# GATB/leon

Hardware: AMD Instinct MI355X
Metric: compressed input MB/s (DNA encode path) (higher is better)
Workload: dtype u64

## Files before the change

### include/leon_dna.h

```cpp
#ifndef LEON_DNA_H
#define LEON_DNA_H

#include <stddef.h>
#include <stdint.h>

#ifdef __cplusplus
extern "C" {
#endif

#define LEON_DNA_ABI_VERSION 5

enum {
    LEON_OK = 0,
    LEON_E_INVALID = -1,
    LEON_E_NO_DEVICE = -2,
    LEON_E_HIP = -3,
    LEON_E_STATE = -4,
    LEON_E_OVERFLOW = -5,
    LEON_E_SINK = -6
};

typedef struct leon_dna_ctx leon_dna_ctx;

typedef struct leon_dna_cfg {
// ... 14 lines not shown
#define LEON_F_DICT_ON_DEVICE 2u

typedef int (*leon_block_sink)(void* user, uint64_t block_id, const uint8_t* payload, uint64_t size,
                               uint32_t n_reads);

typedef struct leon_dna_stats {
    uint64_t n_reads, n_bases, n_blocks, n_anchors, n_no_anchor, n_symbols, payload_bytes;
    uint64_t resolve_rounds, resolve_windows;
    float ms_pack, ms_resolve, ms_sort, ms_walk, ms_symbols, ms_rangecoder, ms_d2h, ms_total;
    uint32_t walk_launches, reserved;
    float ms_anchor_wait, ms_chain_busy;
    float ms_exchange, ms_exchange_call, ms_emulated, ms_emulated_lookups;
    uint64_t xch_words_sent, xch_words_received, walk_reads;
    uint64_t resolve_chain_reads, resolve_chain_windows;
    float ms_resolve_chain, ms_gather_call;
} leon_dna_stats;

int  leon_dna_ctx_create(const leon_dna_cfg* cfg, leon_dna_ctx** out);
void leon_dna_ctx_destroy(leon_dna_ctx* ctx);
const char* leon_last_error(const leon_dna_ctx* ctx);
int  leon_dna_abi_version(void);

int leon_dna_bloom_nbytes(const leon_dna_ctx* ctx, uint64_t* nbytes);
int leon_dna_bloom_upload(leon_dna_ctx* ctx, const uint8_t* bits, uint64_t nbytes);
int leon_dna_bloom_download(leon_dna_ctx* ctx, uint8_t* bits, uint64_t nbytes);
int leon_dna_bloom_clear(leon_dna_ctx* ctx);
int leon_dna_bloom_insert(leon_dna_ctx* ctx, const uint64_t* kmers, uint64_t n);
int leon_dna_bloom_insert_device(leon_dna_ctx* ctx, const uint64_t* d_kmers, uint64_t n);
int leon_dna_bloom_device_ptr(leon_dna_ctx* ctx, void** d_bits, uint64_t* nbytes);
int leon_dna_bloom_upload_device(leon_dna_ctx* ctx, const uint8_t* d_bits, uint64_t nbytes);
// ... 167 lines not shown
```

### leon_amd/capi.py

```python
import ctypes as C
import os
import threading

import numpy as np

_HERE = os.path.dirname(os.path.abspath(__file__))

ABI_VERSION = 5
HEADER_TEXT_DEVICE_CAP = 4096
LEON_F_KEEP_TRACE = 1
LEON_F_DICT_ON_DEVICE = 2


class LeonDnaError(RuntimeError):
    def __init__(self, code, msg):
        super().__init__("leon_dna error %d: %s" % (code, msg))
        self.code = code


def lib_path():
    return os.path.join(_HERE, "lib", "libleon_dna.so")


class _Cfg(C.Structure):
    _fields_ = [("struct_size", C.c_uint32), ("kmer_size", C.c_uint32), ("reads_per_block", C.c_uint32),
                ("bloom_n_hash", C.c_uint32), ("bloom_block_nbits", C.c_uint32), ("device_id", C.c_int32),
                ("bloom_tai", C.c_uint64), ("random_values", C.POINTER(C.c_uint64)), ("resolve_window", C.c_uint64),
                ("flags", C.c_uint32), ("reserved", C.c_uint32)]


class Stats(C.Structure):
    _fields_ = [(n, C.c_uint64) for n in ("n_reads", "n_bases", "n_blocks", "n_anchors", "n_no_anchor", "n_symbols",
                                           "payload_bytes", "resolve_rounds", "resolve_windows")] + \
               [(n, C.c_float) for n in ("ms_pack", "ms_resolve", "ms_sort", "ms_walk", "ms_symbols", "ms_rangecoder",
                                         "ms_d2h", "ms_total")] + \
               [("walk_launches", C.c_uint32), ("reserved", C.c_uint32), ("ms_anchor_wait", C.c_float),
                ("ms_chain_busy", C.c_float)] + \
               [(n, C.c_float) for n in ("ms_exchange", "ms_exchange_call", "ms_emulated", "ms_emulated_lookups")] + \
               [(n, C.c_uint64) for n in ("xch_words_sent", "xch_words_received", "walk_reads", "resolve_chain_reads", "resolve_chain_windows")] + \
               [("ms_resolve_chain", C.c_float), ("ms_gather_call", C.c_float)]

    def as_dict(self):
        return {n: getattr(self, n) for n, _ in self._fields_ if not n.startswith("reserved")}


SINK = C.CFUNCTYPE(C.c_int, C.c_void_p, C.c_uint64, C.POINTER(C.c_uint8), C.c_uint64, C.c_uint32)
EXCHANGE = C.CFUNCTYPE(C.c_int, C.c_void_p, C.c_void_p, C.POINTER(C.c_uint64), C.c_uint32, C.POINTER(C.c_void_p), C.POINTER(C.c_uint64))
XCH_OFF, XCH_BY_ANCHOR, XCH_EMULATE = 0, 1, 2
GATHER = C.CFUNCTYPE(C.c_int, C.c_void_p, C.c_void_p, C.c_uint64, C.c_uint32)

PIECE_SINK = C.CFUNCTYPE(C.c_int, C.c_void_p, C.c_uint64, C.c_void_p, C.c_uint64)


class RecordLayout(C.Structure):
    _fields_ = [("struct_size", C.c_uint32), ("lead", C.c_uint8), ("fastq", C.c_uint8), ("plus_kind", C.c_uint8), ("reserved", C.c_uint8),
# ... 1058 lines not shown
```

### leon_amd/csrc/capi.hip

```cpp
#include "../../include/leon_dna.h"
#include "kernels.h"
#include "host_rc.h"
#include "staging.h"
#include "host_blocks.h"
#include "host_bgzf.h"

#include "prim.h"

#include <algorithm>
#include <atomic>
#include <chrono>
#include <cstdio>
#include <cstdlib>
#include <cstring>
#include <functional>
#include <mutex>
#include <string>
#include <thread>
#include <vector>

using namespace leon;

namespace {

// ... 80 lines not shown
    DevBuf anchor_kmers;
    AnchorDictWorker* anchor_worker = nullptr;
    double anchor_wait_ms = 0;
    std::vector<uint8_t> dict_device_out;
    uint64_t next_read = 0, next_block = 0;
    uint32_t shard_rank = 0, shard_world = 1;
    uint32_t xch_mode = LEON_XCH_OFF;
    leon_exchange_fn xch_fn = nullptr; void* xch_user = nullptr;
    leon_gather_fn gather_fn = nullptr; void* gather_user = nullptr;
    DevBuf xch_slot, xch_off, xch_evoff, xch_events, xch_send, xch_split, xch_res;
    DevBuf resolve_trace;
    DevBuf round_hist;
    DevBuf wcache;
    DevBuf chain_cnt, chain_own, chain_ins, chain_rows, chain_ent, chain_trace, chain_dep, chain_xdep, chain_om, chain_late;
    std::vector<hipEvent_t> chain_ev;
    DevBuf hb_recs[2], hb_recoff, hb_state;
    uint64_t* h_recs = nullptr; size_t h_recs_cap = 0;
    hipStream_t copy_stream = nullptr;
    std::vector<hipEvent_t> hb_ev;
    std::vector<HostBlockCoder> hb_coders;
    uint64_t* h_anchor[2] = {nullptr, nullptr}; size_t h_anchor_cap = 0;
    bool partial_seen = false, finished = false;
    uint64_t hdr_next_read = 0, hdr_next_block = 0;
    bool hdr_partial_seen = false;
    DevBuf hdr_first;
    const uint64_t* walk_keys = nullptr;
    uint32_t fbits_log2 = FBITS_LOG2_DEFAULT;
    bool poisoned = false;
    DevBuf in_bases, in_off, slot_off, packed, nmask, rlen, ncount;
    DevBuf status, hit_pos, hit_slot, cand_pos, cand_slot, anchor_pos, anchor_addr, flags, sort_key, ins_flag, rank;
// ... 461 lines not shown
    }
    CREATE_CHK(c->fbits.ensure((1ull << c->fbits_log2) / 8));
    CREATE_CHK(hipMemsetAsync(c->fbits.p, 0, (1ull << c->fbits_log2) / 8, c->stream));
    CREATE_CHK(hipStreamSynchronize(c->stream));
#undef CREATE_CHK
    c->anchor_worker = new AnchorDictWorker(cfg->kmer_size);
    *out = c;
    return LEON_OK;
}

void leon_dna_ctx_destroy(leon_dna_ctx* c) {
    if (!c) return;
    delete c->anchor_worker;
    (void)hipSetDevice(c->device);
    if (c->stream) (void)hipStreamSynchronize(c->stream);
    dict_free(c->D);
    DevBuf* bufs[] = { &c->anchor_kmers, &c->in_bases, &c->in_off, &c->slot_off, &c->packed, &c->nmask, &c->rlen, &c->ncount,
                       &c->status, &c->hit_pos, &c->hit_slot, &c->cand_pos, &c->cand_slot, &c->anchor_pos, &c->anchor_addr,
                       &c->flags, &c->sort_key, &c->ins_flag, &c->rank, &c->ulist0, &c->ulist1, &c->counters, &c->cub_tmp,
                       &c->sort_key2, &c->perm, &c->perm2, &c->events, &c->prev, &c->sym_off, &c->syms, &c->blk_begin,
                       &c->out_off, &c->out_size, &c->rc_out, &c->rc_scratch, &c->dst_off, &c->payload, &c->errflag, &c->nerr, &c->wbits, &c->fbits, &c->pbits, &c->hdr_first, &c->dc_cache, &c->dc_out, &c->dc_pay, &c->dc_len, &c->dc_pool, &c->dc_scr,
                       &c->xch_slot, &c->xch_off, &c->xch_evoff, &c->xch_events, &c->xch_send, &c->xch_split, &c->xch_res, &c->round_hist, &c->resolve_trace, &c->hb_recs[0], &c->hb_recs[1], &c->hb_recoff, &c->hb_state };
    for (DevBuf* b : bufs) b->release();
    if (c->d_bloom) (void)hipFree(c->d_bloom);
    if (c->d_rv16) (void)hipFree(c->d_rv16);
    if (c->d_nkeys) (void)hipFree(c->d_nkeys);
    if (c->h_payload) (void)hipHostFree(c->h_payload);
    if (c->h_rb) (void)hipHostFree(c->h_rb);
    for (auto& b : c->h_anchor) if (b) (void)hipHostFree(b);
    if (c->h_recs) (void)hipHostFree(c->h_recs);
    for (auto& e : c->hb_ev) (void)hipEventDestroy(e);
    if (c->copy_stream) (void)hipStreamDestroy(c->copy_stream);
    for (auto& e : c->ev) if (e) (void)hipEventDestroy(e);
    for (auto& e : c->pack_ev) (void)hipEventDestroy(e);
    for (auto& e : c->chain_ev) (void)hipEventDestroy(e);
    if (c->stream) (void)hipStreamDestroy(c->stream);
    delete c;
}

int leon_dna_bloom_nbytes(const leon_dna_ctx* c, uint64_t* n) {
    if (!c || !n) return LEON_E_INVALID;
    *n = c->bloom_nchar;
    return LEON_OK;
}
int leon_dna_bloom_upload(leon_dna_ctx* c, const uint8_t* bits, uint64_t n) {
    if (!c || !bits) return LEON_E_INVALID;
    if (n != c->bloom_nchar) return fail(c, LEON_E_INVALID, "bloom_upload: size differs from leon_dna_bloom_nbytes");
    HIPCHK(c, hipSetDevice(c->device));
    HIPCHK(c, staged_h2d(c->device, c->d_bloom, bits, n));
    return LEON_OK;
// ... 72 lines not shown
}
int leon_dna_bloom_contains(leon_dna_ctx* c, const uint64_t* kmers, uint64_t n, uint8_t* out) {
    return bloom_query(c, kmers, n, 0, out);
}

static uint64_t first_window(uint64_t window) { return std::min<uint64_t>(window, 1ull << 17); }
static uint64_t group_end(uint64_t a, uint64_t n, uint64_t window) {
    if (a == 0) return std::min(n, first_window(window));
    return std::min(n, a + 8 * std::min<uint64_t>(window, 1ull << 20));
}

namespace {

struct EncodeKnobs {
    uint32_t rounds_ahead, rounds_max;
    uint32_t chain_chunk;
    bool xch_lookups, walk_cache;
    long walk_cache_log2, walk_hop_log2;
    bool trace_step, trace_resolve, trace_chain;
};
long env_num(const char* name, long dflt) { const char* e = getenv(name); return e ? atol(e) : dflt; }
EncodeKnobs read_encode_knobs() {
    const char* rounds = getenv("LEON_RESOLVE_ROUNDS");
    const long ahead = env_num("LEON_RESOLVE_ROUNDS", 0), most = rounds && strchr(rounds, ':') ? atol(strchr(rounds, ':') + 1) : 0;
    const long chunk = env_num("LEON_CHAIN_CHUNK", 0), hop = env_num("LEON_WALK_HOP_LOG2", 4);
    EncodeKnobs K{};
    K.rounds_ahead = ahead >= 1 && ahead <= 32 ? (uint32_t)ahead : 3u;
    K.rounds_max = std::max<uint32_t>(K.rounds_ahead, most >= 1 && most <= 62 ? (uint32_t)most : 9u);
    K.chain_chunk = chunk >= 1 && chunk <= (1l << CHAIN_LOG2) ? (uint32_t)chunk : 1u << CHAIN_LOG2;
    K.xch_lookups = env_num("LEON_XCH_LOOKUPS", 1) != 0; K.walk_cache = env_num("LEON_WALK_CACHE", 1) != 0;
    K.walk_cache_log2 = env_num("LEON_WALK_CACHE_LOG2", 0); K.walk_hop_log2 = hop >= 1 && hop <= 8 ? hop : 4;
    K.trace_step = getenv("LEON_TRACE_STEP"); K.trace_resolve = getenv("LEON_TRACE_RESOLVE"); K.trace_chain = getenv("LEON_TRACE_CHAIN");
    return K;
}

struct EncodeBatch {
    leon_dna_ctx* const c;
    const uint8_t* const d_bases; const uint64_t* const d_off; const uint64_t n, first_read_index; const leon_block_sink sink; void* const user;
    Upload* const up; const uint64_t* const up_off;
    const uint64_t* const walk_keys = c->walk_keys;
    const EncodeKnobs knobs = read_encode_knobs();
    const std::chrono::steady_clock::time_point t_enter = std::chrono::steady_clock::now();
    const hipStream_t s = c->stream;
    const uint32_t rpb = c->cfg.reads_per_block, k = c->cfg.kmer_size;
    uint64_t n_blocks = 0, off_first = 0, off_last = 0, n_slots = 0, W = 0, KW = 0;
    ReadsDev R{}; ResolveDev V{};
    uint64_t packed_upto = 0; uint32_t n_pack_ev = 0;
    static constexpr uint32_t kRoundsMore = 2, kHist = 64;
    uint32_t* counters = nullptr; uint32_t* lists[2] = {nullptr, nullptr}; uint32_t* d_hist = nullptr; unsigned long long* d_trace = nullptr;
    size_t scan_tmp = 0;
    struct Pending { int buf = -1; uint64_t n = 0; } pending;
    int anchor_buf = 0; bool share_lookups = false;
    uint32_t hint = 0;
    uint32_t n_chain_ev = 0;
    float lk_call_ms = 0, lk_emul_ms = 0;
    Share sh{}; uint64_t nl_bases = 0; bool by_anchor = false;
    WalkCache wc{nullptr, 0, 28, 0};
    std::vector<uint64_t> slice_at, rank_r0, send_counts, send_at; size_t scan_n = 0;
    void mark(const char* what) const {
        if (knobs.trace_step) fprintf(stderr, "[leon step] %-34s %8.2f ms\n", what, std::chrono::duration<double, std::milli>(std::chrono::steady_clock::now() - t_enter).count());
    }
    float ms(int a, int b) const { float v = 0; (void)hipEventElapsedTime(&v, c->ev[a], c->ev[b]); return v; }
    int start() {
        c->stats = leon_dna_stats{}; c->walk_keys = nullptr;
        HIPCHK(c, hipMemcpyAsync(c->h_rb + 0, d_off, 8, hipMemcpyDeviceToHost, s));
        HIPCHK(c, hipMemcpyAsync(c->h_rb + 1, d_off + n, 8, hipMemcpyDeviceToHost, s));
        HIPCHK(c, spin_sync(s));
        off_first = c->h_rb[0]; off_last = c->h_rb[1];
        if (off_last < off_first) return fail(c, LEON_E_INVALID, "offsets are not monotonic");
        n_blocks = (n + rpb - 1) / rpb;
        HIPCHK(c, hipEventRecord(c->ev[0], s));
        HIPCHK(c, c->slot_off.ensure((n + 1) * 8));
// ... 106 lines not shown
            }
            HIPCHK(c, hipStreamSynchronize(s));
            lk_emul_ms += ms_since(t_l0);
        }
        launch_lookup_apply(s, R, c->D, V, w0, w1, s0, s1, first_read_index, xres, lists[0], counters);
        return LEON_OK;
    }
    int fixpoint_rounds(uint64_t w0, uint64_t w1, uint32_t& cnt0) {
        int cur = 0;
        uint32_t n_hist = 1;
        bool first_wait = true;
        for (uint32_t ahead = knobs.rounds_ahead;; ahead = kRoundsMore) {
            for (uint32_t r = 0; r < ahead && n_hist < kHist; r++) {
                const int nxt = cur ^ 1;
                const uint32_t h = std::max<uint32_t>(hint >> (2 * (n_hist - 1) < 31 ? 2 * (n_hist - 1) : 31), 4096);
                HIPCHK(c, hipMemsetAsync(counters + nxt, 0, 4, s));
                launch_check(s, R, c->D, V, first_read_index, lists[cur], counters + cur, h, lists[nxt], counters + nxt);
                HIPCHK(c, hipMemcpyAsync(d_hist + n_hist, counters + nxt, 4, hipMemcpyDeviceToDevice, s));
                launch_reset_tent(s, c->D, V, lists[cur], counters + cur, h);
                launch_propose(s, c->D, V, first_read_index, lists[nxt], counters + nxt, h);
                cur = nxt; n_hist++;
            }
            HIPCHK(c, hipMemcpyAsync(c->h_rb + 8, d_hist, n_hist * 4, hipMemcpyDeviceToHost, s));
            HIPCHK(c, hipMemcpyAsync(c->h_rb + 1, c->D.err, 4, hipMemcpyDeviceToHost, s));
            HIPCHK(c, spin_sync(s));
            if (first_wait) { hand_over(); first_wait = false; }
            if (const int derr = (int)(uint32_t)c->h_rb[1]) {
                HIPCHK(c, hipMemsetAsync(c->D.err, 0, 4, s));
                return fail(c, LEON_E_STATE, derr == 2 ? "the look-ups gathered from the other ranks do not fit this rank's reads or dictionary (were all ranks fed the same batches?)"
                                                       : "anchor dictionary: a two-word key stayed half-written (a stalled wave); batch abandoned");
            }
            const uint32_t* hist = reinterpret_cast<const uint32_t*>(c->h_rb + 8);
            cnt0 = hist[0];
            for (uint32_t r = 1; r < n_hist; r++)
                if (hist[r - 1] > 0 && hist[r] >= hist[r - 1]) return fail(c, LEON_E_STATE, "anchor resolution made no progress (internal error)");
            const uint32_t cnt = hist[n_hist - 1];
            const bool halving = n_hist >= 2 && 2ull * hist[n_hist - 1] <= hist[n_hist - 2];
            if (cnt == 0 || !halving || n_hist - 1 >= knobs.rounds_max || n_hist + kRoundsMore > kHist) {
                for (uint32_t r = 1; r < n_hist; r++) if (hist[r - 1] > 0) c->stats.resolve_rounds++;
                return cnt ? chain_tail(cnt, w0, w1, lists[cur ^ 1]) : LEON_OK;
            }
        }
    }
    int chain_tail(uint32_t left, uint64_t w0, uint64_t w1, uint32_t* clist) {
        if (int rc = event_pair(c, c->chain_ev, n_chain_ev)) return rc;
        HIPCHK(c, hipEventRecord(c->chain_ev[2 * n_chain_ev], s));
        uint32_t* rank = c->rank.as<uint32_t>();
        launch_chain_flags(s, V, w0, w1, V.ins_flag);
        HIPCHK(c, prim::ExclusiveSum(c->cub_tmp.p, scan_tmp, V.ins_flag, rank, w1 - w0, s));
        launch_chain_compact(s, V, w0, w1, rank, clist);
// ... 10 lines not shown
            uint64_t* rows = c->chain_rows.as<uint64_t>();
            uint32_t* cnt = c->chain_cnt.as<uint32_t>(); uint32_t* own = c->chain_own.as<uint32_t>();
            unsigned long long* om = c->chain_om.as<unsigned long long>(); unsigned long long* late = c->chain_late.as<unsigned long long>();
            unsigned long long* dep = c->chain_dep.as<unsigned long long>(); unsigned long long* xdep = c->chain_xdep.as<unsigned long long>();
            size_t rows_tmp = 0;
            HIPCHK(c, prim::ExclusiveSum(nullptr, rows_tmp, rows, rows, nG + 1, s));
            if (rows_tmp > c->cub_tmp.cap) { HIPCHK(c, hipStreamSynchronize(s)); if (int rc = ensure_cub(c, std::max(rows_tmp, scan_tmp))) return rc; }
            launch_chain_prep(s, false, R, c->D, V, first_read_index, w0, clist + c0, nc, c0, rank, cnt, own, nullptr, nullptr, nullptr, nullptr, nullptr, nullptr);
            launch_chain_tables(s, cnt, own, nc, rows, om, late);
            HIPCHK(c, prim::ExclusiveSum(c->cub_tmp.p, rows_tmp, rows, rows, nG + 1, s));
            HIPCHK(c, hipMemcpyAsync(c->h_rb + 0, rows + nG, 8, hipMemcpyDeviceToHost, s));
            HIPCHK(c, spin_sync(s));
            const uint64_t total_rows = c->h_rb[0];
            HIPCHK(c, c->chain_ent.ensure(std::max<uint64_t>(total_rows, 1) * 64 * 4)); uint32_t* ent = c->chain_ent.as<uint32_t>();
            launch_chain_prep(s, true, R, c->D, V, first_read_index, w0, clist + c0, nc, c0, rank, cnt, own, rows, ent, om, late, dep, xdep);
            if (launch_chain_seq(s, nc, cnt, own, dep, xdep, rows, ent, c->chain_ins.as<unsigned long long>(), d_ctrace))
                return fail(c, LEON_E_HIP, "the sequential resolution pass could not be launched (its LDS request was refused)");
            launch_chain_apply(s, c->D, V, first_read_index, clist + c0, nc, c->chain_ins.as<unsigned long long>(), k);
            HIPCHK(c, hipGetLastError());
        }
        { const uint32_t c_last = (left - 1) / CH * CH; launch_chain_repropose(s, c->D, V, first_read_index, clist + c_last, left - c_last, nullptr, 0); }
        HIPCHK(c, hipEventRecord(c->chain_ev[2 * n_chain_ev + 1], s));
        n_chain_ev++;
        c->stats.resolve_chain_reads += left; c->stats.resolve_chain_windows++;
        if (knobs.trace_chain) {
            unsigned long long t[8];
            HIPCHK(c, hipStreamSynchronize(s));
            HIPCHK(c, hipMemcpy(t, d_ctrace, sizeof t, hipMemcpyDeviceToHost));
            float cms = 0; (void)hipEventElapsedTime(&cms, c->chain_ev[2 * n_chain_ev - 2], c->chain_ev[2 * n_chain_ev - 1]);
            fprintf(stderr, "[leon chain] window [%llu, %llu): %u reads left by the rounds; %llu steps of 64, %.2f ballot iterations and %.1f entry rows per step, %llu inserters; %.2f ms; per step the settler waited %.0f (tester: %.0f), settled + published %.0f ticks of s_memtime\n",
// ... 29 lines not shown
            if (w0 == 0) {
                HIPCHK(c, spin_sync(s));
                hand_over();
                mark("first window's anchors to the chain");
            }
        }
        c->n_anchors += n_new;
        return LEON_OK;
    }
    void hand_over() {
        if (pending.buf < 0) return;
        std::vector<uint64_t> fresh(c->h_anchor[pending.buf], c->h_anchor[pending.buf] + pending.n * KW);
        c->anchor_worker->push(std::move(fresh));
        pending.buf = -1;
    }
    int take_share() {
        sh = share_of(c, n);
        uint64_t off_r0 = off_first, off_r1 = off_last;
        if (c->shard_world > 1) {
            HIPCHK(c, hipMemcpy(&off_r0, d_off + sh.r0, 8, hipMemcpyDeviceToHost));
            HIPCHK(c, hipMemcpy(&off_r1, d_off + sh.r0 + sh.nl, 8, hipMemcpyDeviceToHost));
        }
        nl_bases = off_r1 - off_r0;
        R.ev_origin = sh.r0;
        c->stats.n_reads = sh.nl; c->stats.n_bases = nl_bases; c->stats.n_blocks = sh.nbl; c->stats.n_anchors = c->n_anchors;
        c->last_n = n; c->last_bases = nl_bases; c->last_d_bases = d_bases; c->last_d_off = d_off;
        by_anchor = c->shard_world > 1 && c->xch_mode != LEON_XCH_OFF;
        return LEON_OK;
    }
    int walk() {
        HIPCHK(c, c->events.ensure(nl_bases + 16));
        HIPCHK(c, hipMemsetAsync(c->events.p, 0, nl_bases + 16, s));
        start_walk_cache();
        HIPCHK(c, c->perm.ensure(n * 4));
        hipLaunchKernelGGL(k_iota, dim3((uint32_t)std::min<uint64_t>((n + 255) / 256, 8192)), dim3(256), 0, s, c->perm.as<uint32_t>(), n);
        return by_anchor ? walk_by_anchor() : walk_share();
    }
    void start_walk_cache() {
        uint64_t buckets = knobs.walk_cache ? walk_cache_buckets(c) : 0;
        if (!buckets) return;
        if (knobs.walk_cache_log2 >= 10 && knobs.walk_cache_log2 <= 31) buckets = 1ull << knobs.walk_cache_log2;
        size_t free_b = 0, total_b = 0;
        if (hipMemGetInfo(&free_b, &total_b) == hipSuccess) while (buckets > 1024 && buckets * 64 > c->wcache.cap && buckets * 64 > free_b / 8) buckets >>= 1;
        if (c->wcache.ensure(buckets * 64) != hipSuccess) { (void)hipGetLastError(); return; }
        wc.slots = c->wcache.as<uint64_t>(); wc.bucket_mask = buckets - 1; wc.hop_shift = 32 - knobs.walk_hop_log2;
        launch_walk_cache_init(s, wc, k);
    }
    int walk_share() {
        const uint64_t r0 = sh.r0, nl = sh.nl;
        HIPCHK(c, c->sort_key2.ensure(nl * 8)); HIPCHK(c, c->perm2.ensure(nl * 4));
        const uint64_t* walk_key = walk_keys ? walk_keys + r0 : V.sort_key + r0;
        const unsigned key_bits = walk_keys ? 48u : 33u;
        auto sort = [&](void* t, size_t& b) { return prim::SortPairs(t, b, walk_key, c->sort_key2.as<uint64_t>(), c->perm.as<uint32_t>() + r0, c->perm2.as<uint32_t>(), nl, 0, key_bits, s); };
        if (int rc = run_prim(c, sort)) return rc;
        HIPCHK(c, hipEventRecord(c->ev[3], s));
        HIPCHK(c, hipEventRecord(c->ev[4], s));
        launch_walk(s, R, c->B, c->d_rv16, V.anchor_pos, V.flags, c->perm2.as<uint32_t>(), nl, c->events.as<uint8_t>(), nullptr, wc);
        HIPCHK(c, hipEventRecord(c->ev[5], s));
        c->stats.walk_launches = 1; c->stats.walk_reads = nl;
        return LEON_OK;
    }
    int walk_by_anchor() {
        const uint32_t Wd = c->shard_world, me = c->shard_rank;
        if (Wd + 2 > 4096 / 8) return fail(c, LEON_E_INVALID, "set_exchange: world too large");
        if (int rc = cut_slices()) return rc;
        HIPCHK(c, hipMemsetAsync(c->errflag.as<int>() + 1, 0, 4, s));
        const auto t_x0 = std::chrono::steady_clock::now();
        if (int rc = walk_slice(me, true)) return rc;
        HIPCHK(c, hipStreamSynchronize(s));
        float walk_own = 0; (void)hipEventElapsedTime(&walk_own, c->ev[4], c->ev[5]);
        c->stats.xch_words_sent = send_at[Wd];
        if (c->xch_mode == LEON_XCH_BY_ANCHOR) {
            const uint64_t* d_recv = nullptr; uint64_t recv_total = 0;
            const auto t_call = std::chrono::steady_clock::now();
// ... 88 lines not shown
    int code(CodedBlocks& out) {
        HIPCHK(c, c->prev.ensure(n * 8));
        HIPCHK(c, c->nerr.ensure(sh.nl * 8));
        launch_prev_anchored(s, V.anchor_pos, n, rpb, sh.lb0, sh.nbl, c->prev.as<int64_t>());
        auto symbols = [&](uint8_t* syms) {
            launch_symbols(s, R, V.anchor_pos, V.anchor_addr, V.flags, c->prev.as<int64_t>(), c->events.as<uint8_t>(), sh.r0, sh.nl,
                           c->sym_off.as<uint64_t>(), c->nerr.as<uint32_t>(), syms);
        };
        return code_blocks(c, sh, symbols, SMALL_SIZES_DNA, true, "read", out);
    }
    int finish(int last_ev, const CodedBlocks* out = nullptr) {
        leon_dna_stats& st = c->stats;
        const float pack2 = pairs_ms(c->pack_ev, 1, n_pack_ev);
        st.ms_pack = ms(0, 1) + pack2; st.ms_resolve = ms(1, 2) - pack2; st.ms_resolve_chain = pairs_ms(c->chain_ev, 0, n_chain_ev);
        if (last_ev >= 5) { st.ms_sort = ms(2, 3); st.ms_walk = ms(4, 5); }
        if (out) {
            st.n_symbols = out->n_syms; st.payload_bytes = out->payload_bytes;
            st.ms_symbols = by_anchor ? ms(9, 6) : ms(5, 6); st.ms_rangecoder = ms(6, 7); st.ms_d2h = ms(7, 8);
        }
        st.ms_total = ms(0, last_ev);
        if (out) { if (int rc = deliver_blocks(c, *out, sh, n, c->next_block, sink, user)) return rc; }
        c->next_read += n;
        c->next_block += n_blocks;
        if (n % rpb) c->partial_seen = true;
        c->poisoned = false;
        return LEON_OK;
    }
};


// ... 112 lines not shown
    if (int rc = ensure_pack_bufs(c, n, n_slots)) return rc;
    if (int rc = ensure_resolve_bufs(c, n, W)) return rc;
    HIPCHK(c, c->sort_key2.ensure(n * 8)); HIPCHK(c, c->perm.ensure(n * 4)); HIPCHK(c, c->perm2.ensure(n * 4));
    HIPCHK(c, c->events.ensure(max_bases + 16));
    HIPCHK(c, c->prev.ensure(n * 8)); HIPCHK(c, c->sym_off.ensure((n + 1) * 8)); HIPCHK(c, c->nerr.ensure(n * 8));
    HIPCHK(c, c->syms.ensure(est_syms * 2 + 256));
    if (int rc = ensure_block_bufs(c, nbl)) return rc;
    if (int rc = ensure_rc_bufs(c, nbl, est_syms)) return rc;
    HIPCHK(c, c->payload.ensure(max_bases / 12 + 4096));
    size_t t1 = 0, t2 = 0, t3 = 0;
    HIPCHK(c, prim::ExclusiveSum(nullptr, t1, c->slot_off.as<uint64_t>(), c->slot_off.as<uint64_t>(), n + 1, c->stream));
    HIPCHK(c, prim::SortPairs(nullptr, t2, c->sort_key.as<uint64_t>(), c->sort_key2.as<uint64_t>(), c->perm.as<uint32_t>(), c->perm2.as<uint32_t>(),
                                                 n, 0, 33, c->stream));
    HIPCHK(c, prim::ExclusiveSum(nullptr, t3, c->ins_flag.as<uint32_t>(), c->rank.as<uint32_t>(), W, c->stream));
    if (int rc = ensure_cub(c, std::max(t1, std::max(t2, t3)))) return rc;
    if (int rc = ensure_host_payload(c, max_bases / 12 + 4096, max_bases / 12 + 4096)) return rc;
    size_t free_b = 0, total_b = 0;
    if (const uint64_t buckets = walk_cache_buckets(c))
        if (hipMemGetInfo(&free_b, &total_b) == hipSuccess && buckets * 64 <= free_b / 8 && c->wcache.ensure(buckets * 64) != hipSuccess) (void)hipGetLastError();
    if (int rc = dict_reserve(c, c->n_keys + n / 6 + 1024)) return rc;
    if ((n / 6) * 8 * kmer_words(c->cfg.kmer_size) > c->anchor_kmers.cap && c->n_anchors == 0) HIPCHK(c, c->anchor_kmers.ensure((n / 6) * 8 * kmer_words(c->cfg.kmer_size)));
    HIPCHK(c, hipStreamSynchronize(c->stream));
    leon_device_trim();
    return LEON_OK;
}

static int header_batch_impl(leon_dna_ctx* c, const uint8_t* d_hdr, const uint64_t* d_off, uint64_t n, uint64_t first_read_index,
                             const uint8_t* first_header, uint64_t first_len, leon_block_sink sink, void* user) {
    if (!c) return LEON_E_INVALID;
    if (first_read_index != c->hdr_next_read) return fail(c, LEON_E_STATE, "first_read_index does not continue the header stream");
// ... 1034 lines not shown
```

### leon_amd/csrc/dna_kernels.hip

```cpp
#include "kernels.h"

namespace leon {

static inline uint32_t grid_for(uint64_t items, uint32_t per_block, uint32_t cap = 256 * 32) {
    uint64_t g = (items + per_block - 1) / per_block;
    if (g < 1) g = 1;
    if (g > cap) g = cap;
    return (uint32_t)g;
}
#define DISPATCH_K(k, CALL) do { if ((k) >= 32) { typedef u128 K; CALL; } else { typedef uint64_t K; CALL; } } while (0)

template <typename K>
__global__ void __launch_bounds__(256) k_bloom_insert(BloomDev B, const uint16_t* rv16g, const uint64_t* kmers, uint64_t n) {
    __shared__ uint16_t rv16[256];
    load_rv16(rv16, rv16g);
    uint32_t* words = (uint32_t*)B.bits;
    for (uint64_t i = blockIdx.x * (uint64_t)blockDim.x + threadIdx.x; i < n; i += (uint64_t)gridDim.x * blockDim.x) {
        BloomKeys Kk;
        const uint32_t pv = bloom_item_keys<K>(B, rv16, load_kmer<K>(kmers + i * KT<K>::W), Kk);
        for (uint32_t h = 0; h < B.n_hash; h++) {
            uint64_t pos = Kk.racine + Kk.key[h] + pv;
            atomicOr(&words[pos >> 5], 1u << (pos & 31));
        }
    }
// ... 485 lines not shown
        if (want) {
            uint32_t at = block_at + (uint32_t)__popcll(wm & ((1ull << lane) - 1));
            for (uint32_t w = 0; w < wv; w++) at += wave_n[w];
            ulist[at] = (uint32_t)i;
        }
        __syncthreads();
    }
}
void launch_lookup_apply(hipStream_t s, ReadsDev R, DictDev D, ResolveDev V, uint64_t w0, uint64_t w1, uint64_t s0, uint64_t s1,
                         uint64_t first_global, const uint64_t* xres, uint32_t* ulist, uint32_t* ucount) {
    if (w1 - w0 <= s1 - s0) return;
    DISPATCH_K(R.k, hipLaunchKernelGGL(k_lookup_apply<K>, dim3(grid_for((w1 - w0) - (s1 - s0), 256, 256 * 16)), dim3(256), 0, s, R, D, V, w0, w1, s0, s1,
                                       first_global, xres, ulist, ucount));
}

template <typename K>
__global__ void __launch_bounds__(256) k_check(ReadsDev R, DictDev D, ResolveDev V, uint64_t first_global,
                                              const uint32_t* ulist, const uint32_t* ucount,
                                              uint32_t* next_list, uint32_t* next_count) {
    const uint32_t lane = lane_id(), k = R.k;
    const uint32_t grp = lane >> 4, l = lane & 15, gbase = grp * 16;
    const uint64_t wave = (blockIdx.x * (uint64_t)blockDim.x + threadIdx.x) >> 6;
    const uint64_t nwaves = ((uint64_t)gridDim.x * blockDim.x) >> 6;
    const uint32_t count = *ucount;
    __shared__ uint32_t lists[4][64];
    uint32_t* my_list = lists[threadIdx.x >> 6];
    uint32_t n_list = 0;
    auto flush_list = [&]() {
        if (!n_list) return;
        uint32_t at = 0;
        if (lane == 0) at = atomicAdd(next_count, n_list);
        at = (uint32_t)__shfl((int)at, 0);
        __builtin_amdgcn_wave_barrier();
        if (lane < n_list) next_list[at + lane] = my_list[lane];
// ... 53 lines not shown
                const uint32_t wb = window_bit(dict_key<K>(D, slot));
                atomicOr(&D.wbits[wb >> 5], 1u << (wb & 31));
            }
        }
        for (unsigned long long im = __ballot(inserter && l == 0); im; im &= im - 1) {
            const uint32_t src = (uint32_t)__builtin_ctzll(im);
            const uint32_t ii = (uint32_t)__shfl((int)i, (int)src);
            const K key = dict_key<K>(D, V.cand_slot[ii]);
            const uint32_t hmin = key_minimizer_wave(D, key, k, lane);
            if (lane == 0) atomicOr((unsigned long long*)D.fbits + filter_word(D, hmin), (unsigned long long)filter_bits(key));
        }
    }
    flush_list();
}
void launch_check(hipStream_t s, ReadsDev R, DictDev D, ResolveDev V, uint64_t first_global, const uint32_t* ulist,
                  const uint32_t* ucount, uint32_t max_count, uint32_t* next_list, uint32_t* next_count) {
    if (!max_count) return;
    DISPATCH_K(R.k, hipLaunchKernelGGL(k_check<K>, dim3(grid_for(max_count, 16, 256 * 16)), dim3(256), 0, s, R, D, V, first_global, ulist,
                                       ucount, next_list, next_count));
}

__global__ void k_reset_tent(DictDev D, ResolveDev V, const uint32_t* list, const uint32_t* count) {
    uint32_t n = *count;
    for (uint64_t e = blockIdx.x * (uint64_t)blockDim.x + threadIdx.x; e < n; e += (uint64_t)gridDim.x * blockDim.x)
        *tent_ptr(D, V.cand_slot[list[e]]) = IDX_INF;
}
void launch_reset_tent(hipStream_t s, DictDev D, ResolveDev V, const uint32_t* list, const uint32_t* count, uint32_t max_count) {
    if (!max_count) return;
    hipLaunchKernelGGL(k_reset_tent, dim3(grid_for(max_count, 256)), dim3(256), 0, s, D, V, list, count);
}
__global__ void k_propose(DictDev D, ResolveDev V, uint64_t first_global, const uint32_t* list, const uint32_t* count) {
    uint32_t n = *count;
    for (uint64_t e = blockIdx.x * (uint64_t)blockDim.x + threadIdx.x; e < n; e += (uint64_t)gridDim.x * blockDim.x) {
        uint32_t i = list[e];
        atomicMin((unsigned long long*)tent_ptr(D, V.cand_slot[i]), (unsigned long long)(first_global + i));
    }
}
void launch_propose(hipStream_t s, DictDev D, ResolveDev V, uint64_t first_global, const uint32_t* list,
                    const uint32_t* count, uint32_t max_count) {
    if (!max_count) return;
    hipLaunchKernelGGL(k_propose, dim3(grid_for(max_count, 256)), dim3(256), 0, s, D, V, first_global, list, count);
}

template <typename K>
__global__ void __launch_bounds__(256) k_final_pos(ReadsDev R, DictDev D, ResolveDev V, uint64_t w0, uint64_t w1, uint64_t first_global) {
    const uint32_t lane = lane_id(), k = R.k;
    const uint32_t grp = lane >> 4, l = lane & 15, gbase = grp * 16;
    const uint64_t wave = (blockIdx.x * (uint64_t)blockDim.x + threadIdx.x) >> 6;
    const uint64_t nwaves = ((uint64_t)gridDim.x * blockDim.x) >> 6;
    for (uint64_t i0 = w0 + 4 * wave; i0 < w1; i0 += 4 * nwaves) {
        const uint64_t i = i0 + grp;
        const bool have = i < w1;
        const uint8_t st = have ? V.status[i] : (uint8_t)ST_NOANCHOR;
        const bool mine = st == ST_HIT || st == ST_HITNEW;
        const uint64_t g = first_global + i;
        const uint32_t limit = !mine ? 0u : (st == ST_HIT ? V.hit_pos[i] : R.len[i] - k + 1);
// ... 1055 lines not shown
```

### leon_amd/csrc/kernels.h

```cpp
#pragma once
#include <hip/hip_runtime.h>
#include <stdint.h>
#include "leon_device.h"

namespace leon {

struct ReadsDev {
    const uint32_t* packed;
    const uint32_t* nmask;
    const uint64_t* slot_off;
    const uint64_t* base_off;
    const uint32_t* len;
    const uint32_t* n_count;
    uint64_t n;
    uint64_t ev_origin;
    uint32_t k, pad;
};

struct DictDev {
    uint64_t* slots;
    uint64_t* tent;
    uint64_t tstride;
    uint32_t* addr;
    uint64_t mask;
// ... 32 lines not shown
void launch_bloom_query(hipStream_t s, BloomDev B, const uint16_t* rv16, const uint64_t* kmers, uint64_t n,
                        int mode , uint8_t* out);
void launch_rebase_offsets(hipStream_t s, uint64_t* off, uint64_t n, uint64_t base);
void launch_read_slots(hipStream_t s, const uint64_t* base_off, uint64_t n, uint64_t* slots, uint32_t* bad );
void launch_pack(hipStream_t s, const uint8_t* bases, const uint64_t* base_off, const uint64_t* slot_off, uint64_t n,
                 uint32_t* packed, uint32_t* nmask, uint32_t* len, uint32_t* n_count);
void launch_dict_init(hipStream_t s, DictDev D, uint64_t cap, uint32_t W);
void launch_dict_rehash(hipStream_t s, DictDev from, uint64_t from_cap, DictDev to, uint32_t k);
void launch_lookup_cand(hipStream_t s, ReadsDev R, BloomDev B, const uint16_t* rv16, DictDev D, ResolveDev V,
                        uint64_t w0, uint64_t w1, uint64_t first_global, uint32_t* ulist, uint32_t* ucount,
                        unsigned long long* trace = nullptr ,
                        uint64_t* xres = nullptr ,
                        uint64_t xbase = 0, bool dry = false );
void launch_lookup_apply(hipStream_t s, ReadsDev R, DictDev D, ResolveDev V, uint64_t w0, uint64_t w1, uint64_t s0, uint64_t s1,
                         uint64_t first_global, const uint64_t* xres, uint32_t* ulist, uint32_t* ucount);
void launch_check(hipStream_t s, ReadsDev R, DictDev D, ResolveDev V, uint64_t first_global,
                  const uint32_t* ulist, const uint32_t* ucount, uint32_t max_count, uint32_t* next_list, uint32_t* next_count);
void launch_reset_tent(hipStream_t s, DictDev D, ResolveDev V, const uint32_t* list, const uint32_t* count, uint32_t max_count);
void launch_propose(hipStream_t s, DictDev D, ResolveDev V, uint64_t first_global, const uint32_t* list,
                    const uint32_t* count, uint32_t max_count);
void launch_final_pos(hipStream_t s, ReadsDev R, DictDev D, ResolveDev V, uint64_t w0, uint64_t w1, uint64_t first_global);
void launch_ins_flags(hipStream_t s, ResolveDev V, uint64_t w0, uint64_t w1);
void launch_assign_addr(hipStream_t s, DictDev D, ResolveDev V, uint64_t w0, uint64_t w1, const uint32_t* rank,
                        uint64_t addr_base, uint64_t* anchor_kmers, uint32_t k);
constexpr uint32_t CHAIN_LOG2 = 19;
constexpr uint32_t CHAIN_EL = 96;
constexpr uint32_t CHAIN_DEPTH = 3;
void launch_chain_flags(hipStream_t s, ResolveDev V, uint64_t w0, uint64_t w1, uint32_t* flag);
void launch_chain_compact(hipStream_t s, ResolveDev V, uint64_t w0, uint64_t w1, const uint32_t* rank, uint32_t* list);
void launch_chain_repropose(hipStream_t s, DictDev D, ResolveDev V, uint64_t first_global, const uint32_t* reset_list, uint32_t n_reset,
                            const uint32_t* list, uint32_t n);
void launch_chain_prep(hipStream_t s, bool fill, ReadsDev R, DictDev D, ResolveDev V, uint64_t first_global, uint64_t w0, const uint32_t* list,
                       uint32_t n, uint32_t c0, const uint32_t* rank, uint32_t* cnt, uint32_t* own, const uint64_t* gbase, uint32_t* ent,
                       const unsigned long long* om, const unsigned long long* late, unsigned long long* dep, unsigned long long* xdep);
void launch_chain_tables(hipStream_t s, const uint32_t* cnt, const uint32_t* own, uint32_t n, uint64_t* rows ,
// ... 106 lines not shown
```

Before: 20730.

## Overlap settled-read sort/walk with chain resolution on a second stream; gate futile rounds

```diff
diff --git a/include/leon_dna.h b/include/leon_dna.h
--- a/include/leon_dna.h
+++ b/include/leon_dna.h
@@ -52,6 +52,8 @@
     uint64_t xch_words_sent, xch_words_received, walk_reads;
     uint64_t resolve_chain_reads, resolve_chain_windows;
     float ms_resolve_chain, ms_gather_call;
+    uint64_t tail_groups;
+    float ms_tail_overlapped, reserved_tail;
 } leon_dna_stats;
 
 int  leon_dna_ctx_create(const leon_dna_cfg* cfg, leon_dna_ctx** out);
diff --git a/leon_amd/capi.py b/leon_amd/capi.py
--- a/leon_amd/capi.py
+++ b/leon_amd/capi.py
@@ -38,7 +38,8 @@
                 ("ms_chain_busy", C.c_float)] + \
                [(n, C.c_float) for n in ("ms_exchange", "ms_exchange_call", "ms_emulated", "ms_emulated_lookups")] + \
                [(n, C.c_uint64) for n in ("xch_words_sent", "xch_words_received", "walk_reads", "resolve_chain_reads", "resolve_chain_windows")] + \
-               [("ms_resolve_chain", C.c_float), ("ms_gather_call", C.c_float)]
+               [("ms_resolve_chain", C.c_float), ("ms_gather_call", C.c_float)] + \
+               [("tail_groups", C.c_uint64), ("ms_tail_overlapped", C.c_float), ("reserved_tail", C.c_float)]
 
     def as_dict(self):
         return {n: getattr(self, n) for n, _ in self._fields_ if not n.startswith("reserved")}
diff --git a/leon_amd/csrc/capi.hip b/leon_amd/csrc/capi.hip
--- a/leon_amd/csrc/capi.hip
+++ b/leon_amd/csrc/capi.hip
@@ -118,6 +118,10 @@
     DevBuf wcache;
     DevBuf chain_cnt, chain_own, chain_ins, chain_rows, chain_ent, chain_trace, chain_dep, chain_xdep, chain_om, chain_late;
     std::vector<hipEvent_t> chain_ev;
+    hipStream_t stream2 = nullptr;
+    DevBuf cub_tmp2;
+    std::vector<hipEvent_t> group_ev;
+    hipEvent_t settled_ev = nullptr;
     DevBuf hb_recs[2], hb_recoff, hb_state;
     uint64_t* h_recs = nullptr; size_t h_recs_cap = 0;
     hipStream_t copy_stream = nullptr;
@@ -609,13 +613,14 @@
     delete c->anchor_worker;
     (void)hipSetDevice(c->device);
     if (c->stream) (void)hipStreamSynchronize(c->stream);
+    if (c->stream2) (void)hipStreamSynchronize(c->stream2);
     dict_free(c->D);
     DevBuf* bufs[] = { &c->anchor_kmers, &c->in_bases, &c->in_off, &c->slot_off, &c->packed, &c->nmask, &c->rlen, &c->ncount,
                        &c->status, &c->hit_pos, &c->hit_slot, &c->cand_pos, &c->cand_slot, &c->anchor_pos, &c->anchor_addr,
                        &c->flags, &c->sort_key, &c->ins_flag, &c->rank, &c->ulist0, &c->ulist1, &c->counters, &c->cub_tmp,
                        &c->sort_key2, &c->perm, &c->perm2, &c->events, &c->prev, &c->sym_off, &c->syms, &c->blk_begin,
                        &c->out_off, &c->out_size, &c->rc_out, &c->rc_scratch, &c->dst_off, &c->payload, &c->errflag, &c->nerr, &c->wbits, &c->fbits, &c->pbits, &c->hdr_first, &c->dc_cache, &c->dc_out, &c->dc_pay, &c->dc_len, &c->dc_pool, &c->dc_scr,
-                       &c->xch_slot, &c->xch_off, &c->xch_evoff, &c->xch_events, &c->xch_send, &c->xch_split, &c->xch_res, &c->round_hist, &c->resolve_trace, &c->hb_recs[0], &c->hb_recs[1], &c->hb_recoff, &c->hb_state };
+                       &c->xch_slot, &c->xch_off, &c->xch_evoff, &c->xch_events, &c->xch_send, &c->xch_split, &c->xch_res, &c->round_hist, &c->resolve_trace, &c->cub_tmp2, &c->hb_recs[0], &c->hb_recs[1], &c->hb_recoff, &c->hb_state };
     for (DevBuf* b : bufs) b->release();
     if (c->d_bloom) (void)hipFree(c->d_bloom);
     if (c->d_rv16) (void)hipFree(c->d_rv16);
@@ -629,6 +634,9 @@
     for (auto& e : c->ev) if (e) (void)hipEventDestroy(e);
     for (auto& e : c->pack_ev) (void)hipEventDestroy(e);
     for (auto& e : c->chain_ev) (void)hipEventDestroy(e);
+    for (auto& e : c->group_ev) (void)hipEventDestroy(e);
+    if (c->settled_ev) (void)hipEventDestroy(c->settled_ev);
+    if (c->stream2) (void)hipStreamDestroy(c->stream2);
     if (c->stream) (void)hipStreamDestroy(c->stream);
     delete c;
 }
@@ -731,11 +739,14 @@
 
 struct EncodeKnobs {
     uint32_t rounds_ahead, rounds_max;
+    uint32_t skip_below;
     uint32_t chain_chunk;
+    bool tail_overlap;
     bool xch_lookups, walk_cache;
     long walk_cache_log2, walk_hop_log2;
     bool trace_step, trace_resolve, trace_chain;
 };
+constexpr double kSkipBelow = 0.125;
 long env_num(const char* name, long dflt) { const char* e = getenv(name); return e ? atol(e) : dflt; }
 EncodeKnobs read_encode_knobs() {
     const char* rounds = getenv("LEON_RESOLVE_ROUNDS");
@@ -744,7 +755,11 @@
     EncodeKnobs K{};
     K.rounds_ahead = ahead >= 1 && ahead <= 32 ? (uint32_t)ahead : 3u;
     K.rounds_max = std::max<uint32_t>(K.rounds_ahead, most >= 1 && most <= 62 ? (uint32_t)most : 9u);
+    const char* skip = getenv("LEON_RESOLVE_SKIP_BELOW");
+    const double share = skip ? atof(skip) : kSkipBelow;
+    K.skip_below = share > 0 ? (uint32_t)std::lround(std::min(share, 1.0) * 65536.0) : 0u;
     K.chain_chunk = chunk >= 1 && chunk <= (1l << CHAIN_LOG2) ? (uint32_t)chunk : 1u << CHAIN_LOG2;
+    K.tail_overlap = env_num("LEON_TAIL_OVERLAP", 1) != 0;
     K.xch_lookups = env_num("LEON_XCH_LOOKUPS", 1) != 0; K.walk_cache = env_num("LEON_WALK_CACHE", 1) != 0;
     K.walk_cache_log2 = env_num("LEON_WALK_CACHE_LOG2", 0); K.walk_hop_log2 = hop >= 1 && hop <= 8 ? hop : 4;
     K.trace_step = getenv("LEON_TRACE_STEP"); K.trace_resolve = getenv("LEON_TRACE_RESOLVE"); K.trace_chain = getenv("LEON_TRACE_CHAIN");
@@ -773,6 +788,8 @@
     float lk_call_ms = 0, lk_emul_ms = 0;
     Share sh{}; uint64_t nl_bases = 0; bool by_anchor = false;
     WalkCache wc{nullptr, 0, 28, 0};
+    bool share_found = false; uint64_t walked_upto = 0; uint32_t n_groups = 0;
+    ~EncodeBatch() { if (n_groups) (void)hipStreamSynchronize(c->stream2); }
     std::vector<uint64_t> slice_at, rank_r0, send_counts, send_at; size_t scan_n = 0;
     void mark(const char* what) const {
         if (knobs.trace_step) fprintf(stderr, "[leon step] %-34s %8.2f ms\n", what, std::chrono::duration<double, std::milli>(std::chrono::steady_clock::now() - t_enter).count());
@@ -909,11 +926,12 @@
             for (uint32_t r = 0; r < ahead && n_hist < kHist; r++) {
                 const int nxt = cur ^ 1;
                 const uint32_t h = std::max<uint32_t>(hint >> (2 * (n_hist - 1) < 31 ? 2 * (n_hist - 1) : 31), 4096);
+                const RoundGate gate{d_hist, n_hist >= 2 && n_hist <= knobs.rounds_ahead ? knobs.skip_below : 0u};
                 HIPCHK(c, hipMemsetAsync(counters + nxt, 0, 4, s));
-                launch_check(s, R, c->D, V, first_read_index, lists[cur], counters + cur, h, lists[nxt], counters + nxt);
+                launch_check(s, R, c->D, V, first_read_index, lists[cur], counters + cur, h, lists[nxt], counters + nxt, gate);
                 HIPCHK(c, hipMemcpyAsync(d_hist + n_hist, counters + nxt, 4, hipMemcpyDeviceToDevice, s));
-                launch_reset_tent(s, c->D, V, lists[cur], counters + cur, h);
-                launch_propose(s, c->D, V, first_read_index, lists[nxt], counters + nxt, h);
+                launch_reset_tent(s, c->D, V, lists[cur], counters + cur, h, gate);
+                launch_propose(s, c->D, V, first_read_index, lists[nxt], counters + nxt, h, gate);
                 cur = nxt; n_hist++;
             }
             HIPCHK(c, hipMemcpyAsync(c->h_rb + 8, d_hist, n_hist * 4, hipMemcpyDeviceToHost, s));
@@ -927,8 +945,17 @@
             }
             const uint32_t* hist = reinterpret_cast<const uint32_t*>(c->h_rb + 8);
             cnt0 = hist[0];
+            if (knobs.trace_resolve) {
+                fprintf(stderr, "[leon resolve] window [%llu, %llu): the list after look-ups and rounds:", (unsigned long long)w0, (unsigned long long)w1);
+                for (uint32_t r = 0; r < n_hist; r++) fprintf(stderr, " %u", hist[r]);
+                fprintf(stderr, "\n");
+            }
             for (uint32_t r = 1; r < n_hist; r++)
                 if (hist[r - 1] > 0 && hist[r] >= hist[r - 1]) return fail(c, LEON_E_STATE, "anchor resolution made no progress (internal error)");
+            if (n_hist > 2 && n_hist == 1 + knobs.rounds_ahead && rounds_futile(hist[0], hist[1], knobs.skip_below)) {
+                c->stats.resolve_rounds++;
+                return chain_tail(hist[1], w0, w1, lists[0]);
+            }
             const uint32_t cnt = hist[n_hist - 1];
             const bool halving = n_hist >= 2 && 2ull * hist[n_hist - 1] <= hist[n_hist - 2];
             if (cnt == 0 || !halving || n_hist - 1 >= knobs.rounds_max || n_hist + kRoundsMore > kHist) {
@@ -969,6 +996,7 @@
             const uint64_t total_rows = c->h_rb[0];
             HIPCHK(c, c->chain_ent.ensure(std::max<uint64_t>(total_rows, 1) * 64 * 4)); uint32_t* ent = c->chain_ent.as<uint32_t>();
             launch_chain_prep(s, true, R, c->D, V, first_read_index, w0, clist + c0, nc, c0, rank, cnt, own, rows, ent, om, late, dep, xdep);
+            if (c0 == 0 && w0 > 0 && 8ull * left >= w1 - w0 && groups_allowed()) { if (int rc = walk_group(w0)) return rc; }
             if (launch_chain_seq(s, nc, cnt, own, dep, xdep, rows, ent, c->chain_ins.as<unsigned long long>(), d_ctrace))
                 return fail(c, LEON_E_HIP, "the sequential resolution pass could not be launched (its LDS request was refused)");
             launch_chain_apply(s, c->D, V, first_read_index, clist + c0, nc, c->chain_ins.as<unsigned long long>(), k);
@@ -1028,7 +1056,8 @@
         c->anchor_worker->push(std::move(fresh));
         pending.buf = -1;
     }
-    int take_share() {
+    int find_share() {
+        if (share_found) return LEON_OK;
         sh = share_of(c, n);
         uint64_t off_r0 = off_first, off_r1 = off_last;
         if (c->shard_world > 1) {
@@ -1037,20 +1066,30 @@
         }
         nl_bases = off_r1 - off_r0;
         R.ev_origin = sh.r0;
+        share_found = true;
+        return LEON_OK;
+    }
+    int take_share() {
+        if (int rc = find_share()) return rc;
         c->stats.n_reads = sh.nl; c->stats.n_bases = nl_bases; c->stats.n_blocks = sh.nbl; c->stats.n_anchors = c->n_anchors;
         c->last_n = n; c->last_bases = nl_bases; c->last_d_bases = d_bases; c->last_d_off = d_off;
         by_anchor = c->shard_world > 1 && c->xch_mode != LEON_XCH_OFF;
         return LEON_OK;
     }
     int walk() {
+        if (n_groups) return walk_rest();
+        if (int rc = prepare_walk(s)) return rc;
+        return by_anchor ? walk_by_anchor() : walk_share();
+    }
+    int prepare_walk(hipStream_t st) {
         HIPCHK(c, c->events.ensure(nl_bases + 16));
-        HIPCHK(c, hipMemsetAsync(c->events.p, 0, nl_bases + 16, s));
-        start_walk_cache();
+        HIPCHK(c, hipMemsetAsync(c->events.p, 0, nl_bases + 16, st));
+        start_walk_cache(st);
         HIPCHK(c, c->perm.ensure(n * 4));
-        hipLaunchKernelGGL(k_iota, dim3((uint32_t)std::min<uint64_t>((n + 255) / 256, 8192)), dim3(256), 0, s, c->perm.as<uint32_t>(), n);
-        return by_anchor ? walk_by_anchor() : walk_share();
-    }
-    void start_walk_cache() {
+        hipLaunchKernelGGL(k_iota, dim3((uint32_t)std::min<uint64_t>((n + 255) / 256, 8192)), dim3(256), 0, st, c->perm.as<uint32_t>(), n);
+        return LEON_OK;
+    }
+    void start_walk_cache(hipStream_t st) {
         uint64_t buckets = knobs.walk_cache ? walk_cache_buckets(c) : 0;
         if (!buckets) return;
         if (knobs.walk_cache_log2 >= 10 && knobs.walk_cache_log2 <= 31) buckets = 1ull << knobs.walk_cache_log2;
@@ -1058,20 +1097,61 @@
         if (hipMemGetInfo(&free_b, &total_b) == hipSuccess) while (buckets > 1024 && buckets * 64 > c->wcache.cap && buckets * 64 > free_b / 8) buckets >>= 1;
         if (c->wcache.ensure(buckets * 64) != hipSuccess) { (void)hipGetLastError(); return; }
         wc.slots = c->wcache.as<uint64_t>(); wc.bucket_mask = buckets - 1; wc.hop_shift = 32 - knobs.walk_hop_log2;
-        launch_walk_cache_init(s, wc, k);
+        launch_walk_cache_init(st, wc, k);
+    }
+    int sort_and_walk(hipStream_t st, DevBuf& tmp, uint64_t a, uint64_t m, hipEvent_t e_sorted, hipEvent_t e_walk0, hipEvent_t e_walk1) {
+        const uint64_t at = a - sh.r0;
+        const uint64_t* walk_key = walk_keys ? walk_keys + a : V.sort_key + a;
+        const unsigned key_bits = walk_keys ? 48u : 33u;
+        auto sort = [&](void* t, size_t& b) { return prim::SortPairs(t, b, walk_key, c->sort_key2.as<uint64_t>() + at, c->perm.as<uint32_t>() + a, c->perm2.as<uint32_t>() + at, m, 0, key_bits, st); };
+        if (m) {
+            size_t bytes = 0;
+            HIPCHK(c, sort(nullptr, bytes));
+            HIPCHK(c, tmp.ensure(bytes));
+            HIPCHK(c, sort(tmp.p, bytes));
+        }
+        HIPCHK(c, hipEventRecord(e_sorted, st));
+        HIPCHK(c, hipEventRecord(e_walk0, st));
+        launch_walk(st, R, c->B, c->d_rv16, V.anchor_pos, V.flags, c->perm2.as<uint32_t>() + at, m, c->events.as<uint8_t>(), nullptr, wc);
+        HIPCHK(c, hipEventRecord(e_walk1, st));
+        return LEON_OK;
     }
     int walk_share() {
-        const uint64_t r0 = sh.r0, nl = sh.nl;
-        HIPCHK(c, c->sort_key2.ensure(nl * 8)); HIPCHK(c, c->perm2.ensure(nl * 4));
-        const uint64_t* walk_key = walk_keys ? walk_keys + r0 : V.sort_key + r0;
-        const unsigned key_bits = walk_keys ? 48u : 33u;
-        auto sort = [&](void* t, size_t& b) { return prim::SortPairs(t, b, walk_key, c->sort_key2.as<uint64_t>(), c->perm.as<uint32_t>() + r0, c->perm2.as<uint32_t>(), nl, 0, key_bits, s); };
-        if (int rc = run_prim(c, sort)) return rc;
-        HIPCHK(c, hipEventRecord(c->ev[3], s));
-        HIPCHK(c, hipEventRecord(c->ev[4], s));
-        launch_walk(s, R, c->B, c->d_rv16, V.anchor_pos, V.flags, c->perm2.as<uint32_t>(), nl, c->events.as<uint8_t>(), nullptr, wc);
-        HIPCHK(c, hipEventRecord(c->ev[5], s));
-        c->stats.walk_launches = 1; c->stats.walk_reads = nl;
+        HIPCHK(c, c->sort_key2.ensure(sh.nl * 8)); HIPCHK(c, c->perm2.ensure(sh.nl * 4));
+        if (int rc = sort_and_walk(s, c->cub_tmp, sh.r0, sh.nl, c->ev[3], c->ev[4], c->ev[5])) return rc;
+        c->stats.walk_launches = 1; c->stats.walk_reads = sh.nl;
+        return LEON_OK;
+    }
+    bool groups_allowed() const {
+        return knobs.tail_overlap && !walk_keys && !(c->shard_world > 1 && c->xch_mode != LEON_XCH_OFF) && share_of(c, n).nl > 0;
+    }
+    int walk_group(uint64_t upto) {
+        if (int rc = find_share()) return rc;
+        const uint64_t a = n_groups ? walked_upto : sh.r0, b = std::min(sh.r0 + sh.nl, upto / rpb * rpb);
+        if (b <= a) return LEON_OK;
+        if (!n_groups) {
+            if (!c->stream2) HIPCHK(c, hipStreamCreateWithFlags(&c->stream2, hipStreamNonBlocking));
+            if (!c->settled_ev) HIPCHK(c, hipEventCreateWithFlags(&c->settled_ev, hipEventDisableTiming));
+            HIPCHK(c, c->sort_key2.ensure(sh.nl * 8)); HIPCHK(c, c->perm2.ensure(sh.nl * 4));
+            if (int rc = prepare_walk(c->stream2)) return rc;
+        }
+        while (c->group_ev.size() < 3 * (size_t)(n_groups + 1)) { hipEvent_t e; HIPCHK(c, hipEventCreate(&e)); c->group_ev.push_back(e); }
+        hipEvent_t* ge = c->group_ev.data() + 3 * (size_t)n_groups;
+        HIPCHK(c, hipEventRecord(c->settled_ev, s));
+        HIPCHK(c, hipStreamWaitEvent(c->stream2, c->settled_ev, 0));
+        HIPCHK(c, hipEventRecord(ge[0], c->stream2));
+        n_groups++;
+        if (int rc = sort_and_walk(c->stream2, c->cub_tmp2, a, b - a, ge[1], ge[1], ge[2])) return rc;
+        HIPCHK(c, hipGetLastError());
+        walked_upto = b;
+        return LEON_OK;
+    }
+    int walk_rest() {
+        HIPCHK(c, hipStreamWaitEvent(s, c->group_ev[3 * (size_t)n_groups - 1], 0));
+        HIPCHK(c, hipEventRecord(c->ev[10], s));
+        const uint64_t a = walked_upto;
+        if (int rc = sort_and_walk(s, c->cub_tmp, a, sh.r0 + sh.nl - a, c->ev[3], c->ev[4], c->ev[5])) return rc;
+        c->stats.walk_launches = n_groups + 1; c->stats.walk_reads = sh.nl;
         return LEON_OK;
     }
     int walk_by_anchor() {
@@ -1190,6 +1270,18 @@
         const float pack2 = pairs_ms(c->pack_ev, 1, n_pack_ev);
         st.ms_pack = ms(0, 1) + pack2; st.ms_resolve = ms(1, 2) - pack2; st.ms_resolve_chain = pairs_ms(c->chain_ev, 0, n_chain_ev);
         if (last_ev >= 5) { st.ms_sort = ms(2, 3); st.ms_walk = ms(4, 5); }
+        if (n_groups) {
+            auto at = [&](hipEvent_t e) { float v = 0; (void)hipEventElapsedTime(&v, c->ev[0], e); return v; };
+            st.ms_sort = ms(10, 3);
+            std::vector<std::pair<float, float>> passes(n_chain_ev);
+            for (uint32_t j = 0; j < n_chain_ev; j++) passes[j] = {at(c->chain_ev[2 * j]), at(c->chain_ev[2 * j + 1])};
+            for (uint32_t g = 0; g < n_groups; g++) {
+                const float t0 = at(c->group_ev[3 * g]), t1 = at(c->group_ev[3 * g + 1]), t2 = at(c->group_ev[3 * g + 2]);
+                st.ms_sort += t1 - t0; st.ms_walk += t2 - t1;
+                for (const auto& p : passes) st.ms_tail_overlapped += std::max(0.f, std::min(t2, p.second) - std::max(t0, p.first));
+            }
+            st.tail_groups = n_groups + 1;
+        }
         if (out) {
             st.n_symbols = out->n_syms; st.payload_bytes = out->payload_bytes;
             st.ms_symbols = by_anchor ? ms(9, 6) : ms(5, 6); st.ms_rangecoder = ms(6, 7); st.ms_d2h = ms(7, 8);
@@ -1332,6 +1424,7 @@
                                                  n, 0, 33, c->stream));
     HIPCHK(c, prim::ExclusiveSum(nullptr, t3, c->ins_flag.as<uint32_t>(), c->rank.as<uint32_t>(), W, c->stream));
     if (int rc = ensure_cub(c, std::max(t1, std::max(t2, t3)))) return rc;
+    HIPCHK(c, c->cub_tmp2.ensure(t2));
     if (int rc = ensure_host_payload(c, max_bases / 12 + 4096, max_bases / 12 + 4096)) return rc;
     size_t free_b = 0, total_b = 0;
     if (const uint64_t buckets = walk_cache_buckets(c))
diff --git a/leon_amd/csrc/dna_kernels.hip b/leon_amd/csrc/dna_kernels.hip
--- a/leon_amd/csrc/dna_kernels.hip
+++ b/leon_amd/csrc/dna_kernels.hip
@@ -523,10 +523,13 @@
                                        first_global, xres, ulist, ucount));
 }
 
+__device__ __forceinline__ bool gate_closed(RoundGate g) { return g.below && rounds_futile(g.hist[0], g.hist[1], g.below); }
+
 template <typename K>
 __global__ void __launch_bounds__(256) k_check(ReadsDev R, DictDev D, ResolveDev V, uint64_t first_global,
                                               const uint32_t* ulist, const uint32_t* ucount,
-                                              uint32_t* next_list, uint32_t* next_count) {
+                                              uint32_t* next_list, uint32_t* next_count, RoundGate gate) {
+    if (gate_closed(gate)) return;
     const uint32_t lane = lane_id(), k = R.k;
     const uint32_t grp = lane >> 4, l = lane & 15, gbase = grp * 16;
     const uint64_t wave = (blockIdx.x * (uint64_t)blockDim.x + threadIdx.x) >> 6;
@@ -610,22 +613,24 @@
     flush_list();
 }
 void launch_check(hipStream_t s, ReadsDev R, DictDev D, ResolveDev V, uint64_t first_global, const uint32_t* ulist,
-                  const uint32_t* ucount, uint32_t max_count, uint32_t* next_list, uint32_t* next_count) {
+                  const uint32_t* ucount, uint32_t max_count, uint32_t* next_list, uint32_t* next_count, RoundGate gate) {
     if (!max_count) return;
     DISPATCH_K(R.k, hipLaunchKernelGGL(k_check<K>, dim3(grid_for(max_count, 16, 256 * 16)), dim3(256), 0, s, R, D, V, first_global, ulist,
-                                       ucount, next_list, next_count));
-}
-
-__global__ void k_reset_tent(DictDev D, ResolveDev V, const uint32_t* list, const uint32_t* count) {
+                                       ucount, next_list, next_count, gate));
+}
+
+__global__ void k_reset_tent(DictDev D, ResolveDev V, const uint32_t* list, const uint32_t* count, RoundGate gate) {
+    if (gate_closed(gate)) return;
     uint32_t n = *count;
     for (uint64_t e = blockIdx.x * (uint64_t)blockDim.x + threadIdx.x; e < n; e += (uint64_t)gridDim.x * blockDim.x)
         *tent_ptr(D, V.cand_slot[list[e]]) = IDX_INF;
 }
-void launch_reset_tent(hipStream_t s, DictDev D, ResolveDev V, const uint32_t* list, const uint32_t* count, uint32_t max_count) {
+void launch_reset_tent(hipStream_t s, DictDev D, ResolveDev V, const uint32_t* list, const uint32_t* count, uint32_t max_count, RoundGate gate) {
     if (!max_count) return;
-    hipLaunchKernelGGL(k_reset_tent, dim3(grid_for(max_count, 256)), dim3(256), 0, s, D, V, list, count);
-}
-__global__ void k_propose(DictDev D, ResolveDev V, uint64_t first_global, const uint32_t* list, const uint32_t* count) {
+    hipLaunchKernelGGL(k_reset_tent, dim3(grid_for(max_count, 256)), dim3(256), 0, s, D, V, list, count, gate);
+}
+__global__ void k_propose(DictDev D, ResolveDev V, uint64_t first_global, const uint32_t* list, const uint32_t* count, RoundGate gate) {
+    if (gate_closed(gate)) return;
     uint32_t n = *count;
     for (uint64_t e = blockIdx.x * (uint64_t)blockDim.x + threadIdx.x; e < n; e += (uint64_t)gridDim.x * blockDim.x) {
         uint32_t i = list[e];
@@ -633,9 +638,9 @@
     }
 }
 void launch_propose(hipStream_t s, DictDev D, ResolveDev V, uint64_t first_global, const uint32_t* list,
-                    const uint32_t* count, uint32_t max_count) {
+                    const uint32_t* count, uint32_t max_count, RoundGate gate) {
     if (!max_count) return;
-    hipLaunchKernelGGL(k_propose, dim3(grid_for(max_count, 256)), dim3(256), 0, s, D, V, first_global, list, count);
+    hipLaunchKernelGGL(k_propose, dim3(grid_for(max_count, 256)), dim3(256), 0, s, D, V, first_global, list, count, gate);
 }
 
 template <typename K>
diff --git a/leon_amd/csrc/kernels.h b/leon_amd/csrc/kernels.h
--- a/leon_amd/csrc/kernels.h
+++ b/leon_amd/csrc/kernels.h
@@ -70,11 +70,15 @@
                         uint64_t xbase = 0, bool dry = false );
 void launch_lookup_apply(hipStream_t s, ReadsDev R, DictDev D, ResolveDev V, uint64_t w0, uint64_t w1, uint64_t s0, uint64_t s1,
                          uint64_t first_global, const uint64_t* xres, uint32_t* ulist, uint32_t* ucount);
+struct RoundGate { const uint32_t* hist; uint32_t below; };
+__host__ __device__ inline bool rounds_futile(uint32_t len, uint32_t left, uint32_t below) {
+    return below && (uint64_t)(len - left) * 65536u < (uint64_t)below * len;
+}
 void launch_check(hipStream_t s, ReadsDev R, DictDev D, ResolveDev V, uint64_t first_global,
-                  const uint32_t* ulist, const uint32_t* ucount, uint32_t max_count, uint32_t* next_list, uint32_t* next_count);
-void launch_reset_tent(hipStream_t s, DictDev D, ResolveDev V, const uint32_t* list, const uint32_t* count, uint32_t max_count);
+                  const uint32_t* ulist, const uint32_t* ucount, uint32_t max_count, uint32_t* next_list, uint32_t* next_count, RoundGate gate);
+void launch_reset_tent(hipStream_t s, DictDev D, ResolveDev V, const uint32_t* list, const uint32_t* count, uint32_t max_count, RoundGate gate);
 void launch_propose(hipStream_t s, DictDev D, ResolveDev V, uint64_t first_global, const uint32_t* list,
-                    const uint32_t* count, uint32_t max_count);
+                    const uint32_t* count, uint32_t max_count, RoundGate gate);
 void launch_final_pos(hipStream_t s, ReadsDev R, DictDev D, ResolveDev V, uint64_t w0, uint64_t w1, uint64_t first_global);
 void launch_ins_flags(hipStream_t s, ResolveDev V, uint64_t w0, uint64_t w1);
 void launch_assign_addr(hipStream_t s, DictDev D, ResolveDev V, uint64_t w0, uint64_t w1, const uint32_t* rank,
```

Result: no change. 20820, median of 3 (+0.4%).
